# willi-menapace/PlayableVideoGeneration

Measured on AMD Instinct MI355X. Metric: training clips/sec (B x16x256x256), higher is better.
Workload: dtype f32; 1 GPU; bair256_t16_b8; variant=main, per_gpu_batch=8, global_batch=8, seq_len=16, gt_init=6, parallelism=dp1

## Files before the change

### include/caddy_hip.h

```cpp
#ifndef CADDY_HIP_H
#define CADDY_HIP_H
#include <stddef.h>
#ifdef __cplusplus
extern "C" {
#endif

typedef struct caddy_ctx caddy_ctx;

typedef struct caddy_config {
    int variant;
    int batch;
    int seq_len;
    int height, width;
    int stacking;
    int actions;
    int action_dim;
    int hidden;
    int use_gumbel, hard_gumbel, use_variations;
    float centroid_alpha;
    int perceptual;
    int ensemble;
} caddy_config;
#define CADDY_MAX_ENSEMBLE 8

// ... 123 lines not shown
int caddy_adam_step_ex(caddy_ctx* ctx, float* m, float* v, float lr, float beta1, float beta2, float eps, float weight_decay, int step, const int* member_step, int s2h_step,
                       float grad_scale);

int caddy_start_inference(caddy_ctx* ctx);
int caddy_f16_saturated(caddy_ctx* ctx);
int caddy_fallback_layers(caddy_ctx* ctx);
int caddy_generate_next(caddy_ctx* ctx, const float* observation, int action, const float* variation, float* frame_out, float* obs_out);

#define CADDY_PROFILE_FAMILIES 18
int caddy_debug_set_poison(caddy_ctx* ctx, int on);
int caddy_debug_set_seeds_only(caddy_ctx* ctx, int on);
int caddy_profile_begin(caddy_ctx* ctx);
int caddy_profile_end(caddy_ctx* ctx, double* out );
int caddy_profile_records(caddy_ctx* ctx, double* out, int max_records);
int caddy_profile_phases(caddy_ctx* ctx, char* names_out, float* ms_out, int max);

int caddy_debug_count(caddy_ctx* ctx);
int caddy_debug_fusion_counts(caddy_ctx* ctx, long* out3);
int caddy_debug_set_bn_paths(caddy_ctx* ctx, int small, int lazy, int epilogue_stats);
int caddy_debug_set_vgg_s16(caddy_ctx* ctx, int on);
int caddy_debug_set_s16_grads(caddy_ctx* ctx, int on);
int caddy_debug_set_perc_chunks(caddy_ctx* ctx, int n);
int caddy_debug_set_perc_fuse_l1(caddy_ctx* ctx, int on);
long caddy_debug_s16_grad_count(caddy_ctx* ctx);
int caddy_debug_set_pack_merged(caddy_ctx* ctx, int on);
int caddy_debug_dims(caddy_ctx* ctx, int i, int* nhwc4);
int caddy_debug_get(caddy_ctx* ctx, int i, int grad, float* dst_nchw);

int caddy_bn_layer_count(caddy_ctx* ctx);
long caddy_bn_calls(caddy_ctx* ctx, int i, char* name_out128);

struct ConvArgs; struct WgradArgs; struct PackDesc; struct TV;
int caddy_k_conv_fwd(const struct ConvArgs* a, void* stream);
int caddy_k_conv_wgrad(const struct WgradArgs* a, void* stream);
struct IgemmArgs;
size_t caddy_k_igemm_weight_bytes(int Cin, int Cout, int KH, int KW);
int caddy_k_igemm_pack(const float* w, const float* gamma, const float* beta, const float* mean, const float* var, float eps, const float* bias_in, int Cin, int Cout, int KH, int KW,
                       void* w32, void* w16, float* bias_out, void* stream);
int caddy_k_conv_igemm(const struct IgemmArgs* a, void* stream);
int caddy_k_fid_pool(const struct TV* in, const struct TV* out, int mode, void* stream);
int caddy_k_fid_global_avg(const struct TV* in, double* out, void* stream);
int caddy_k_fid_stage(const float* src, int n, int Hs, int Ws, float* out, int Ho, int Wo, void* stream);
struct Conv3dArgs; struct V5;
size_t caddy_k_conv3d_weight_bytes(int Cin, int Cout, int KT, int KH, int KW);
int caddy_k_conv3d_pack(const float* w_dhwio, const float* gamma, const float* beta, const float* mean, const float* var, float eps, const float* bias_in, int Cin, int Cout, int KT, int KH,
                        int KW, void* w32, void* w16, float* bias_out, void* stream);
// ... 25 lines not shown
```

### playablevideogeneration_amd/_lib.py

```python
import ctypes as C
import os

HERE = os.path.dirname(os.path.abspath(__file__))
LIB_PATH = os.path.join(HERE, "csrc", "libcaddy_hip.so")
CONV_MAX_SRC = 3
CONV_BK = 16


class TV(C.Structure):
    _fields_ = [("p", C.c_void_p), ("N", C.c_int), ("H", C.c_int), ("W", C.c_int), ("C", C.c_int), ("sn", C.c_long), ("ld", C.c_int), ("s16", C.c_int)]


class ConvSrc(C.Structure):
    _fields_ = [("p", C.c_void_p), ("sn", C.c_long), ("ld", C.c_int), ("C", C.c_int), ("Cpad", C.c_int), ("bcast", C.c_int),
                ("bn_scale", C.c_void_p), ("bn_shift", C.c_void_p), ("bn_act", C.c_int), ("bn_gn", C.c_int), ("bn_gs", C.c_long)]


class ConvArgs(C.Structure):
    _fields_ = [("src", ConvSrc * CONV_MAX_SRC), ("nsrc", C.c_int), ("N", C.c_int), ("H", C.c_int), ("W", C.c_int), ("KS", C.c_int),
                ("wp", C.c_void_p), ("Ktot", C.c_int), ("Cout", C.c_int), ("Cout_pad", C.c_int), ("bias", C.c_void_p), ("act", C.c_int),
                ("out", C.c_void_p), ("out_sn", C.c_long), ("out_ld", C.c_int), ("accumulate", C.c_int), ("precision", C.c_int), ("splitk", C.c_int), ("aux", C.c_void_p), ("split_scratch", C.c_void_p), ("split_cap", C.c_long), ("split_stride", C.c_long),
                ("mask", C.c_void_p), ("seed_ref", C.c_void_p), ("seed_w", C.c_float), ("wq", C.c_void_p), ("Kq", C.c_int), ("out_scale", C.c_float),
                ("res", C.c_void_p), ("res_sn", C.c_long), ("res_ld", C.c_int), ("xcd_map", C.c_int),
                ("pool_out", C.c_void_p), ("pool_sn", C.c_long), ("pool_ld", C.c_int), ("skip_out", C.c_int),
                ("stats", C.c_void_p), ("stats_ld", C.c_int), ("sat_flag", C.c_void_p), ("deterministic", C.c_int), ("direct_ok", C.c_int), ("lstm", C.c_void_p),
                ("in_s16", C.c_int), ("out_s16", C.c_int), ("pool_s16", C.c_int), ("mask_s16", C.c_int), ("seed_s16", C.c_int),
                ("avgpool", C.c_int), ("sat_out_next", C.c_int),
                ("l1_acc", C.c_void_p)]


class LstmFuse(C.Structure):
    _fields_ = [("cprev", C.c_void_p), ("cprev_sn", C.c_long), ("cprev_ld", C.c_int), ("h", C.c_void_p), ("h_sn", C.c_long), ("h_ld", C.c_int),
                ("c", C.c_void_p), ("c_sn", C.c_long), ("c_ld", C.c_int), ("hb", C.c_void_p), ("hb_sn", C.c_long), ("hb_ld", C.c_int),
                ("scale", C.c_void_p), ("shift", C.c_void_p), ("C", C.c_int)]


class WgradArgs(C.Structure):
    _fields_ = [("src", ConvSrc * CONV_MAX_SRC), ("nsrc", C.c_int), ("N", C.c_int), ("H", C.c_int), ("W", C.c_int), ("KS", C.c_int),
                ("dy", C.c_void_p), ("dy_sn", C.c_long), ("dy_ld", C.c_int), ("Cout", C.c_int), ("Cout_pad", C.c_int), ("Ktot", C.c_int),
                ("dwp", C.c_void_p), ("slabs", C.c_int), ("group_n", C.c_int), ("src_gs", C.c_long * CONV_MAX_SRC), ("dy_gs", C.c_long), ("precision", C.c_int),
                ("src_bn_gs", C.c_long * CONV_MAX_SRC), ("det_slab", C.c_void_p), ("det_cap", C.c_long), ("det_stride", C.c_long), ("dy_s16", C.c_int)]


class PackDesc(C.Structure):
    _fields_ = [("w", C.c_void_p * 4), ("gw", C.c_void_p * 4), ("nw", C.c_int), ("Co_each", C.c_int), ("Cin", C.c_int), ("KS", C.c_int),
                ("nseg", C.c_int), ("seg_off", C.c_int * CONV_MAX_SRC), ("seg_C", C.c_int * CONV_MAX_SRC), ("seg_Cpad", C.c_int * CONV_MAX_SRC),
                ("Cout", C.c_int), ("Cout_pad", C.c_int), ("Ktot", C.c_int), ("oscale", C.c_void_p)]


def round_up(a, b):
    return (a + b - 1) // b * b


_lib = None


def load(path=None):
    global _lib
    if path is None and _lib is not None:
        return _lib
    p = path or os.environ.get("CADDY_HIP_LIB") or LIB_PATH
    if not os.path.exists(p):
        raise RuntimeError(f"{p} not found: the HIP extension is not built (run __graft_entry__.build()); "
                           "playablevideogeneration_amd has no CPU fallback")
    lib = C.CDLL(p)
    if path is None:
        _lib = lib
    return lib
```

### playablevideogeneration_amd/csrc/common.h

```cpp
#pragma once
#include <hip/hip_runtime.h>
#include <cstdint>

typedef float f32x16 __attribute__((ext_vector_type(16)));
typedef float f32x4 __attribute__((ext_vector_type(4)));
typedef __bf16 bf16x8 __attribute__((ext_vector_type(8)));
typedef __bf16 bf16x4 __attribute__((ext_vector_type(4)));

struct TV {
    float* p;
    int N, H, W, C;
    long sn;
    int ld;
    int s16;
};

static inline int cdiv(long a, long b) { return (int)((a + b - 1) / b); }
static inline int round_up(int a, int b) { return (a + b - 1) / b * b; }

#define CONV_MAX_SRC 3
#define CONV_BK 16
struct ConvSrc {
    const float* p;
    long sn;
// ... 35 lines not shown
    int Kq;
    float out_scale;
    const float* res;
    long res_sn;
    int res_ld;
    int xcd_map;
    float* pool_out;
    long pool_sn;
    int pool_ld;
    int skip_out;
    float* stats;
    int stats_ld;
    unsigned* sat_flag;
    int deterministic;
    int direct_ok;
    const struct LstmFuse* lstm;
    int in_s16;
    int out_s16;
    int pool_s16;
    int mask_s16, seed_s16;
    int avgpool;
    int sat_out_next;
    double* l1_acc;
};
int conv_avgpool_ok(const ConvArgs& a);
struct LstmFuse { const float* cprev; long cprev_sn; int cprev_ld; float* h; long h_sn; int h_ld; float* c; long c_sn; int c_ld; float* hb; long hb_sn; int hb_ld; const float* scale; const float* shift; int C; };
extern thread_local int g_last_conv_lstm_fused;
#define HX_WSCALE 64.0f
enum { PREC_FP32 = 0, PREC_F16X3 = 16, PREC_BF16X3 = 17, PREC_F16X1 = 18, PREC_BF16X1 = 19 };
#define HX_KC 32
constexpr int CONV_AUX_BYTES = 128 * 1024;

struct WgradArgs {
    ConvSrc src[CONV_MAX_SRC];
    int nsrc;
    int N, H, W;
    int KS;
    const float* dy;
    long dy_sn;
    int dy_ld;
    int Cout, Cout_pad;
    int Ktot;
    float* dwp;
    int slabs;
    int group_n;
    long src_gs[CONV_MAX_SRC];
// ... 57 lines not shown
```

### playablevideogeneration_amd/csrc/conv_hx.hip

```cpp
#include "conv_hx_common.h"
#include "pack.h"
#include "pack_elems.h"
#include <cstdlib>

namespace {

template <typename T> __device__ __forceinline__ unsigned s16_bits(T h) { unsigned short s; __builtin_memcpy(&s, &h, 2); return s; }
template <typename T> __device__ __forceinline__ unsigned s16_pair(float v, int lane) {
    const T hi = (T)v;
    const T lo = (T)(v - (float)hi);
    const unsigned u = s16_bits(hi) | (s16_bits(lo) << 16);
    const unsigned w = (unsigned)__builtin_amdgcn_mov_dpp((int)u, 0xB1 , 0xF, 0xF, true);
    return (lane & 1) ? ((w >> 16) | (u & 0xffff0000u)) : ((u & 0xffffu) | (w << 16));
}
__device__ __forceinline__ int s16_slot(int col) { return (col & ~31) | ((col & 31) >> 1) | ((col & 1) << 4); }
__device__ __forceinline__ float s16_hi(const float* row, int col) { return (float)reinterpret_cast<const _Float16*>(row + (col & ~31))[col & 31]; }
__device__ __forceinline__ float s16_val(const float* row, int col) {
    const _Float16* h = reinterpret_cast<const _Float16*>(row + (col & ~31));
    return (float)h[col & 31] + (float)h[32 + (col & 31)];
}

template <typename T, int TH, int TW, int BN, int WM, int WN, int EP, bool SO, bool INTR, int MODE, int TMt, int TNt>
__device__ __forceinline__ void hx_epilogue(f32x16 (&acc)[TMt][TNt], float (&st1)[TNt], float (&st2)[TNt], unsigned& amax_o, double& l1s, const ConvArgs& a,
                                            int n, int n0, int y0, int x0, int lane, int wave) {
    constexpr bool E_POOL = EP == 1 || EP == 3, E_MASK = EP == 2 || EP == 3;
    constexpr int BM = TH * TW, RW = BM / WM / TW;
    const int wm_u = __builtin_amdgcn_readfirstlane(wave) / WN, wn = wave % WN;
    const int yw = y0 + wm_u * RW, xl = x0 + 4 * (lane >> 5);
    const int nx = a.W - xl;
    const bool masked = MODE == 1 || MODE == 3 || (MODE == 2 && E_MASK && a.mask != nullptr);
    const bool split = MODE == 2 && a.splitk > 1, slabs = split && a.split_stride != 0, atomics = split && !slabs;
    const bool with_res = MODE == 2 && !split && a.res != nullptr, accum = MODE == 2 && !split && a.accumulate != 0;
    char* const op = reinterpret_cast<char*>(a.out + (long)n * a.out_sn + (slabs ? (long)blockIdx.z * a.split_stride : 0L));
    const char* const mp = masked ? reinterpret_cast<const char*>(a.mask + (long)n * a.out_sn) : nullptr;
    const char* const sp = (masked && a.seed_ref) ? reinterpret_cast<const char*>(a.seed_ref + (long)n * a.out_sn) : nullptr;
    const char* const rp = with_res ? reinterpret_cast<const char*>(a.res + (long)n * a.res_sn) : nullptr;
    const unsigned ldb = (unsigned)a.out_ld * 4u, wldb = (unsigned)a.W * ldb;
// ... 62 lines not shown
                        if (EP == 0 && !split) { st1[j] += v; st2[j] = fmaf(v, v, st2[j]); }
                        const unsigned o_ = cb + HX_EOFF(i, r, wldb, ldb);
                        if (SO) {
                            if (!is_bf16<T>::value) { amax_o = max(amax_o, __float_as_uint(v) & 0x7fffffffu); v = __builtin_amdgcn_fmed3f(v, -HX_F16_MAX, HX_F16_MAX); if (E_POOL) acc[i][j][r] = v; }
                            const unsigned w_ = s16_pair<T>(v, lane);
                            if (store_full) *reinterpret_cast<unsigned*>(op + o_) = w_;
                        } else if (atomics) atomicAdd(reinterpret_cast<float*>(op + o_), v);
                        else if (store_full) *reinterpret_cast<float*>(op + o_) = v;
                    }
                }
                if (E_POOL && a.pool_out) {
                    char* const pp = reinterpret_cast<char*>(a.pool_out + (long)n * a.pool_sn);
                    const unsigned plb = (unsigned)a.pool_ld * 4u;
                    const int py = (yw + i * 2) >> 1;
                    const unsigned pb0 = (unsigned)(py * (a.W >> 1) + (xl >> 1)) * plb + ((SO && a.pool_s16) ? (unsigned)s16_slot(col) : (unsigned)col) * 4u;
#pragma unroll
                    for (int r = 0; r < 8; r += 2) {
                        const int pdx = ((r & 3) + 8 * ((r >> 2) & 1)) >> 1;
                        if (!INTR && (py >= (a.H >> 1) || (xl >> 1) + pdx >= (a.W >> 1))) continue;
                        const float mx = fmaxf(fmaxf(acc[i][j][r], acc[i][j][r + 1]), fmaxf(acc[i][j][r + 8], acc[i][j][r + 9]));
                        const unsigned po_ = pb0 + (unsigned)pdx * plb;
                        if (SO && a.pool_s16) *reinterpret_cast<unsigned*>(pp + po_) = s16_pair<T>(mx, lane);
                        else *reinterpret_cast<float*>(pp + po_) = mx;
                    }
                }
            }
        }
    }
#undef HX_EOFF
#undef HX_EOK
}

template <typename T, int NPL, int TH, int TW, int BN, int WM, int WN, int D, int EP = 0, int IO = 0, int BG = 0>
__global__ __launch_bounds__(64 * WM * WN) void k_conv_hx(ConvArgs a, int tiles_x, int tiles_y) {
    typedef typename Vec<T>::v8 v8;
    typedef typename Vec<T>::v4 v4;
    constexpr int NT = 64 * WM * WN;
    constexpr bool E_POOL = EP == 1 || EP == 3, E_MASK = EP == 2 || EP == 3;
    constexpr bool PS = (IO & 1) != 0, SO = (IO & 2) != 0;
    static_assert(!(PS || SO) || NPL == 2, "S16 tensors carry both halves");
    constexpr int BM = TH * TW;
    constexpr int HW_ = TW + 2, HH_ = TH + 2, HPX = HW_ * HH_;
    constexpr int PITCH = NPL * KC + 8;
    constexpr int AROW = (HW_ * PITCH + 127) / 128 * 128;
    constexpr int APP = NT / 8;
    constexpr int NA = (HPX + APP - 1) / APP;
// ... 484 lines not shown
    return true;
}
thread_local int g_last_conv_stats_tiles = 0;
thread_local int g_last_conv_direct = 0;

int conv_hx_avgpool_ok(const ConvArgs& a0) {
    ConvArgs a = a0;
    a.avgpool = 1;
    return conv_hx_try(a, nullptr, true) == 1 ? 1 : 0;
}

int conv_hx_try(const ConvArgs& a0, hipStream_t st, bool dry) {
    ConvArgs a = a0;
    if (a.KS != 3 || !a.wq || a.precision < PREC_F16X3 || a.precision > PREC_BF16X1 || a.act == 1) return 0;
    int kq = 0;
    for (int s = 0; s < a.nsrc; s++) { if ((a.src[s].ld & 3) || (a.src[s].sn & 3)) return -1; kq += round_up(a.src[s].C, HX_KC); }
    a.Kq = kq;
    a.out_scale = (a.precision == PREC_F16X3 || a.precision == PREC_F16X1) ? 1.0f / HX_WSCALE : 1.0f;
    int bn = hx_pick_bn(a.Cout);
    a.Cout_pad = round_up(a.Cout, bn);
    if (a.mask && a.accumulate) return -1;
    if (a.l1_acc && !conv_hx_l1_ok(a)) return -1;
    if (a.pool_out && (a.accumulate || a.mask)) return -1;
    if (a.avgpool) {
        if ((a.H | a.W) & 1 || a.accumulate || a.mask || a.pool_out || a.skip_out || a.stats || a.lstm || a.precision != PREC_F16X3 || a.in_s16 || a.out_s16) return dry ? 0 : -1;
        if (a.direct_ok && conv_direct_try(a, st, dry) == 1) {
            if (!dry) { g_last_conv_kernel = CK_HX_32; g_last_conv_stats_tiles = 0; g_last_conv_direct = 1; }
            return 1;
        }
    }
    if ((long)a.H * a.W * a.out_ld >= (1L << 30) || (a.res && (long)a.H * a.W * a.res_ld >= (1L << 30))) return 0;
    const int nchunks = kq / HX_KC;
    if (bn == 128 && g_hx_big_override < 0 && !a.pool_out && !a.skip_out && !a.mask &&
        (long)a.N * cdiv(a.W, 16) * cdiv(a.H, 8) * (a.Cout_pad / 128) <= 256) bn = 64;
    const int force_big = g_hx_big_override;
    bool big = bn == 128 && (long)a.N * cdiv(a.W, 16) * cdiv(a.H, 16) * (a.Cout_pad / bn) >= 384;
    if (force_big >= 0) big = bn == 128 && force_big == 1;
    const bool small_tiles = bn < 128 && force_big != 1 && (long)a.N * cdiv(a.W, 16) * cdiv(a.H, 16) * (a.Cout_pad / bn) < 384;
    const long blocks8 = (long)a.N * cdiv(a.W, 16) * cdiv(a.H, 8) * (a.Cout_pad / bn);
    const bool th4 = bn == 64 && small_tiles && !a.pool_out && !a.skip_out && !a.mask && !a.stats && blocks8 < 200 &&
                     ((a.direct_ok && a.precision == PREC_F16X3 && !a.accumulate) || a.precision == PREC_BF16X3);
    const int th = th4 ? 4 : ((bn == 128 && !big) || small_tiles) ? 8 : 16;
    const int tx = cdiv(a.W, 16), ty = cdiv(a.H, th);
    const long blocks = (long)a.N * tx * ty * (a.Cout_pad / bn);
    g_last_conv_direct = 0;
    if (!dry && !a.avgpool && a.direct_ok && blocks < 200 && conv_direct_try(a, st) == 1) { g_last_conv_kernel = CK_HX_32; g_last_conv_stats_tiles = 0; g_last_conv_direct = 1; return 1; }
// ... 107 lines not shown
```

### playablevideogeneration_amd/csrc/net.cpp

```cpp
#include "net.h"
#include "fid.h"
#include "fvd.h"
#include <cmath>
#include <cstdio>
#include <cstdlib>
#include <cstring>

static thread_local std::string g_err;
int finish(caddy_ctx* c, const char* sizer) {
    if (!c->dry && c->act.overflow() && !c->fail) { c->fail = true; g_err = std::string("activation arena overflow (workspace smaller than ") + sizer + ")"; }
    if (!c->dry) {
        hipError_t e = hipGetLastError();
        if (e != hipSuccess && !c->fail) { c->fail = true; g_err = std::string("HIP error: ") + hipGetErrorString(e); }
    }
    return c->fail ? -1 : 0;
}
void set_error(const std::string& s) { g_err = s; }
extern "C" const char* caddy_last_error(void) { return g_err.c_str(); }

#define RUN(expr) do { if (!dry) ck((expr), #expr); } while (0)

void caddy_ctx::ck(int rc, const char* what) {
    if (rc != 0 && !fail) { fail = true; set_error(std::string("kernel launch failed: ") + what); }
}
// ... 1451 lines not shown
    delete c;
}
size_t caddy_workspace_bytes(const caddy_config* cfg) {
    if (!check_cfg(cfg)) return 0;
    size_t p, a; dry_sizes(cfg, &p, &a);
    return p + 2 * a + 4096;
}
caddy_ctx* caddy_ctx_create(const caddy_config* cfg, float* params, float* grads, void* workspace, size_t workspace_bytes) {
    if (!check_cfg(cfg)) return nullptr;
    if (!params || !grads || !workspace) { set_error("null buffer"); return nullptr; }
    size_t p, a; dry_sizes(cfg, &p, &a);
    if (workspace_bytes < p + 2 * a) { set_error("workspace too small (see caddy_workspace_bytes)"); return nullptr; }
    if (((uintptr_t)workspace & 255) || ((uintptr_t)params & 15) || ((uintptr_t)grads & 15)) { set_error("buffers must be 256-byte (workspace) / 16-byte (params, grads) aligned"); return nullptr; }
    caddy_ctx* c = make_ctx(cfg, params, grads, workspace, a);
    if (c->fail) { delete c; return nullptr; }
    if (caddy_serial_streams()) c->use_dstream = false;
    hipMemset(c->sat_flag, 0, sizeof(unsigned) * 2 * CADDY_N_FLAGS);
    if (const char* e = getenv("CADDY_DETERMINISTIC")) c->deterministic = atoi(e) != 0;
    if (const char* e = getenv("CADDY_PERC_CHUNKS")) { const int n = atoi(e); if (n < 0) c->perc_chunks_force = -n; else c->perc_chunks_cfg = n; }
    if (const char* e = getenv("CADDY_MASK_FROM_X")) c->mask_from_x = atoi(e) != 0;
    if (const char* e = getenv("CADDY_S16_GRADS")) c->s16_grads = atoi(e) != 0;
    if (const char* e = getenv("CADDY_VGG_S16")) c->vgg_s16 = atoi(e) != 0;
    if (const char* e = getenv("CADDY_PERC_FUSE_L1")) c->perc_fuse_l1 = atoi(e) != 0;
    if (const char* e = getenv("CADDY_PRECISION")) {
        if (!strcmp(e, "exact") || !strcmp(e, "0")) { c->prec_fwd = c->prec_bwd = PREC_FP32; c->vgg_precision = c->vgg_precision_bwd = PREC_FP32; }
        else if (!strcmp(e, "fwd")) { c->prec_bwd = PREC_FP32; c->vgg_precision_bwd = PREC_FP32; }
    }
    return c;
}
extern "C" int caddy_dp_shutdown(caddy_ctx* c);
void caddy_ctx_destroy(caddy_ctx* c) {
    if (c && (c->comm || c->comm2)) caddy_dp_shutdown(c);
    if (c && c->side) { hipStreamSynchronize(c->side); hipStreamDestroy(c->side); }
    if (c) for (int k = 0; k < caddy_ctx::PERC_MAX_CHUNKS; k++) if (c->perc_ev[k]) hipEventDestroy(c->perc_ev[k]);
    if (c && c->gstream) { if (c->graph_exec) hipStreamSynchronize(c->stream); hipStreamSynchronize(c->gstream); c->drop_graph(); hipStreamDestroy(c->gstream); }
    if (c) for (ConvL* L : c->convs) if (L->off_ev) hipEventDestroy(L->off_ev);
    if (c && c->dstream) { hipStreamSynchronize(c->dstream); hipStreamDestroy(c->dstream); if (c->d_done) hipEventDestroy(c->d_done); }
    fid_free(c);
    fvd_free(c);
    delete c;
}
int caddy_set_stream(caddy_ctx* c, void* s) { c->stream = (hipStream_t)s; return 0; }
int caddy_debug_set_poison(caddy_ctx* c, int on) { c->poison_nz = on != 0; return 0; }
int caddy_debug_set_bn_paths(caddy_ctx* c, int small, int lazy, int epilogue_stats) { c->bn_small = small != 0; c->lazy_bn = lazy != 0; c->epi_stats = epilogue_stats != 0; return 0; }
int caddy_debug_set_vgg_s16(caddy_ctx* c, int on) { c->vgg_s16 = on != 0; return 0; }
int caddy_debug_set_s16_grads(caddy_ctx* c, int on) { c->s16_grads = on != 0; return 0; }
int caddy_debug_set_perc_chunks(caddy_ctx* c, int n) { c->perc_chunks_force = n; return 0; }
int caddy_debug_set_perc_fuse_l1(caddy_ctx* c, int on) { c->perc_fuse_l1 = on != 0; return 0; }
long caddy_debug_s16_grad_count(caddy_ctx* c) { long n = 0; for (const GradFmt& g : c->gfmts) n += g.fmt ? 1 : 0; return n; }
int caddy_debug_set_pack_merged(caddy_ctx* c, int on) { c->merged_pack = on != 0; c->pack_jobs.key = -1; for (auto& j : c->unpack_jobs) j.key = -1; return 0; }
int caddy_debug_set_seeds_only(caddy_ctx* c, int on) { c->seeds_only = on != 0; return 0; }
int caddy_set_grads_ready_hook(caddy_ctx* c, caddy_grads_ready_hook hook, void* user) { c->grads_hook = hook; c->grads_user = user; return 0; }
int caddy_set_sampler_hook(caddy_ctx* c, caddy_sampler_hook hook, void* user, int provides_samples, int provides_variations) {
    c->samplers = SamplerHooks{};
    if (hook && (provides_samples || provides_variations)) { c->samplers.fn = hook; c->samplers.user = user; c->samplers.action = provides_samples; c->samplers.variation = provides_variations; }
    return 0;
}
int caddy_set_allreduce_hook(caddy_ctx* c, void (*hook)(float*, int, void*), void* user, int world_size) {
    c->hook = hook; c->hook_user = user; c->world = world_size > 1 ? world_size : 1;
    return 0;
}
int caddy_forward_full(caddy_ctx* c, const float* obs, int gt_init, float tau, const caddy_noise* noise, int training, const float* samples_in, const float* variations_in) {
    if (!ctx_needs(c, CTX_MODEL, "caddy_forward_full")) return -2;
    c->fail = false;
    if (!obs || !noise) { set_error("null input"); return -2; }
    return forward_full(c, obs, gt_init, tau, noise, training, samples_in, variations_in);
}
int caddy_forward_pretraining(caddy_ctx* c, const float* obs, float tau, const caddy_noise* noise, int training, const float* samples_in, const float* variations_in) {
    if (!ctx_needs(c, CTX_MODEL, "caddy_forward_pretraining")) return -2;
    c->fail = false;
    if (!obs || !noise) { set_error("null input"); return -2; }
// ... 166 lines not shown
```

### playablevideogeneration_amd/csrc/net.h

```cpp
#pragma once
#include <algorithm>
#include <array>
#include <deque>
#include <functional>
#include <string>
#include <vector>
#include "caddy_hip.h"
#include "common.h"
#include "head.h"
#include "pack.h"
#include "pointwise.h"
#include "perceptual.h"

struct GradFmt { bool elig; int fmt; };
struct T4 {
    float* d; float* g;
    int N, H, W, C; long sn; int ld;
    bool nz = false;
    bool nz2 = false;
    const float* bn_scale = nullptr; const float* bn_shift = nullptr; int bn_act = 0;
    int fmt = 0;
    GradFmt* gs = nullptr;
};
static inline TV dv(const T4& t) { return TV{t.d, t.N, t.H, t.W, t.C, t.sn, t.ld, 0}; }
// ... 111 lines not shown
    void (*grads_hook)(float* grads, long offset, long count, void* stream, void* user) = nullptr; void* grads_user = nullptr;
    long bucket_lo[2] = {0, 0}, bucket_hi[2] = {0, 0}; bool lstm_early_done = false;
    long s2h_lo = 0, s2h_hi = 0;
    void early_gradient_buckets();
    void* comm = nullptr; void* comm2 = nullptr;
    int comm_world = 1; std::vector<std::pair<long, long>> comm_buckets; hipStream_t comm_bucket_stream = nullptr;
    SamplerHooks samplers{};
    bool deterministic = true;
    float* wgrad_det = nullptr; long wgrad_det_cap = 0;
    hipStream_t wgrad_det_owner = nullptr; bool wgrad_det_owner_set = false;
    long n_pool_fallback = 0;
    long n_wgrad_det_handover = 0;
    unsigned* sat_flag = nullptr;
    bool layer_fallback[CADDY_N_FLAGS] = {false};
    int n_fallback = 0;
    float* conv_split = nullptr; long conv_split_cap = 0;
    float* conv_aux = nullptr;
    float* conv_aux2 = nullptr;
    double* red_scratch = nullptr;
    VggState vgg;
    int vgg_precision = PREC_F16X3, vgg_precision_bwd = PREC_BF16X3;
    bool vgg_s16 = true;
    bool perc_fuse_l1 = true;
    int prec_fwd = PREC_F16X3, prec_bwd = PREC_BF16X3;
    T4 gt_img[3]{}; size_t gt_scratch_off = 0, gt_scratch_end = 0; bool gt_prefetched = false, perc_prefetch = true; hipEvent_t gt_done = nullptr;
    static constexpr int PERC_MAX_CHUNKS = 8;
    int perc_chunks_cfg = 3;
    int perc_chunks_force = 0;
    int perc_nch = 1, perc_trec = 0;
    int perc_t0[PERC_MAX_CHUNKS + 1] = {};
    hipEvent_t perc_ev[PERC_MAX_CHUNKS] = {};
    bool perc_waited[PERC_MAX_CHUNKS] = {};
    bool perc_pipelined = false;
    T4 gt_taps_c[PERC_MAX_CHUNKS][3][5]{};
    bool perc_range(int r, int k, int* t0, int* len) const {
        if (r == 0 || perc_nch == 1) { if (r != 0 && k != 0) return false; *t0 = r == 0 ? perc_t0[k + 1] : 0; *len = r == 0 ? perc_t0[k] - perc_t0[k + 1] : perc_trec; return true; }
        const int kb = perc_nch / 2;
        if (k == 0) { *t0 = perc_t0[kb]; *len = perc_trec - perc_t0[kb]; return true; }
        if (k == kb) { *t0 = 0; *len = perc_t0[kb]; return true; }
        return false;
    }
    void perc_plan(int Trec, bool chunked);
    void perc_wait(int t);
    size_t gt_lo = 0, gt_hi = 0;
    size_t fwd_off = 0;
    int prof_kind_override = -1;
// ... 93 lines not shown
```

### playablevideogeneration_amd/csrc/perceptual.hip

```cpp
#include "net.h"
#include "perceptual.h"
#include "lpips.h"
#include <cstdio>
#include <cstring>

#define RUN_CK(c, expr) do { if (!(c)->dry) (c)->ck((expr), #expr); } while (0)

namespace {

const VggSpec VGG19_SPEC[VGG_NCONV] = {
    {0, 3, 64, 0, 0}, {2, 64, 64, 0, -1}, {5, 64, 128, 1, 1}, {7, 128, 128, 0, -1}, {10, 128, 256, 1, 2}, {12, 256, 256, 0, -1}, {14, 256, 256, 0, -1},
    {16, 256, 256, 0, -1}, {19, 256, 512, 1, 3}, {21, 512, 512, 0, -1}, {23, 512, 512, 0, -1}, {25, 512, 512, 0, -1}, {28, 512, 512, 1, 4}};
const VggSpec LPIPS_SPEC[VGG_NCONV] = {
    {0, 3, 64, 0, -1}, {2, 64, 64, 0, 0}, {5, 64, 128, 1, -1}, {7, 128, 128, 0, 1}, {10, 128, 256, 1, -1}, {12, 256, 256, 0, -1}, {14, 256, 256, 0, 2},
    {17, 256, 512, 1, -1}, {19, 512, 512, 0, -1}, {21, 512, 512, 0, 3}, {24, 512, 512, 1, -1}, {26, 512, 512, 0, -1}, {28, 512, 512, 0, 4}};
const int LPIPS_C[5] = {64, 128, 256, 512, 512};

__global__ __launch_bounds__(256) void k_maxpool2(const float* in, float* out, long n_out4, int Hi, int Wi, int C4) {
    const int Ho = Hi >> 1, Wo = Wi >> 1;
    for (long i = blockIdx.x * 256L + threadIdx.x; i < n_out4; i += (long)gridDim.x * 256) {
        int c = (int)(i % C4); long q = i / C4; int x = (int)(q % Wo); q /= Wo; int y = (int)(q % Ho); long n = q / Ho;
        const float4* p = reinterpret_cast<const float4*>(in) + ((n * Hi + 2 * y) * (long)Wi + 2 * x) * C4 + c;
        float4 a = p[0], b = p[C4], d = p[(long)Wi * C4], e = p[(long)Wi * C4 + C4];
        float4 m;
// ... 30 lines not shown
}
template <bool AS, bool ZS>
__global__ __launch_bounds__(256) void k_maxpool2_bwd_relu(const float* a, const float* gp, float* gz, long n_win4, int Hi, int Wi, int C4) {
    const int Ho = Hi >> 1, Wo = Wi >> 1, Hc = (Hi + 1) >> 1, Wc = (Wi + 1) >> 1;
    for (long i = blockIdx.x * 256L + threadIdx.x; i < n_win4; i += (long)gridDim.x * 256) {
        int c = (int)(i % C4); long q = i / C4; int x = (int)(q % Wc); q /= Wc; int y = (int)(q % Hc); long n = q / Hc;
        const long base = ((n * Hi + 2 * y) * (long)Wi + 2 * x) * C4 + c;
        const long o1 = C4, o2 = (long)Wi * C4, o3 = o2 + C4;
        if (y >= Ho || x >= Wo) {
            const float4 zero = make_float4(0.f, 0.f, 0.f, 0.f);
            st4_grad<ZS>(gz, base, zero);
            if (2 * x + 1 < Wi) st4_grad<ZS>(gz, base + o1, zero);
            if (2 * y + 1 < Hi) { st4_grad<ZS>(gz, base + o2, zero); if (2 * x + 1 < Wi) st4_grad<ZS>(gz, base + o3, zero); }
            continue;
        }
        const float4 A = ld4<AS>(a, base), B = ld4<AS>(a, base + o1), D = ld4<AS>(a, base + o2), E = ld4<AS>(a, base + o3);
        const float4 G = reinterpret_cast<const float4*>(gp)[((n * Ho + y) * (long)Wo + x) * C4 + c];
        float4 zA, zB, zD, zE;
        route4(A.x, B.x, D.x, E.x, G.x, zA.x, zB.x, zD.x, zE.x);
        route4(A.y, B.y, D.y, E.y, G.y, zA.y, zB.y, zD.y, zE.y);
        route4(A.z, B.z, D.z, E.z, G.z, zA.z, zB.z, zD.z, zE.z);
        route4(A.w, B.w, D.w, E.w, G.w, zA.w, zB.w, zD.w, zE.w);
        st4_grad<ZS>(gz, base, zA); st4_grad<ZS>(gz, base + o1, zB); st4_grad<ZS>(gz, base + o2, zD); st4_grad<ZS>(gz, base + o3, zE);
    }
}
template <bool RS, bool GS, bool ZS>
__global__ __launch_bounds__(256) void k_feat_l1(const float* rec, const float* gt, long n4, float seed_w, float* gz, double* acc) {
    __shared__ double sh[4];
    double s = 0.0;
    for (long i = blockIdx.x * 256L + threadIdx.x; i < n4; i += (long)gridDim.x * 256) {
        const float4 r = ld4<RS>(rec, i), g = ld4<GS>(gt, i);
        const float d[4] = {r.x - g.x, r.y - g.y, r.z - g.z, r.w - g.w};
        const float rv[4] = {r.x, r.y, r.z, r.w};
        float z[4];
#pragma unroll
        for (int e = 0; e < 4; e++) {
            s += (double)fabsf(d[e]);
            z[e] = rv[e] > 0.f ? (d[e] > 0.f ? seed_w : (d[e] < 0.f ? -seed_w : 0.f)) : 0.f;
        }
        if (gz) st4_grad<ZS>(gz, i, make_float4(z[0], z[1], z[2], z[3]));
    }
    for (int o = 32; o > 0; o >>= 1) s += __shfl_xor(s, o);
    if ((threadIdx.x & 63) == 0) sh[threadIdx.x >> 6] = s;
    __syncthreads();
    if (threadIdx.x == 0) atomicAdd(acc, sh[0] + sh[1] + sh[2] + sh[3]);
}
// ... 110 lines not shown
    const float* r = rec.d; const float* t = gt.d;
    if (rec.fmt && gt.fmt) hipLaunchKernelGGL((k_feat_l1_img<true, true>), g, b, 0, st, r, t, n4, acc);
    else if (rec.fmt) hipLaunchKernelGGL((k_feat_l1_img<true, false>), g, b, 0, st, r, t, n4, acc);
    else if (gt.fmt) hipLaunchKernelGGL((k_feat_l1_img<false, true>), g, b, 0, st, r, t, n4, acc);
    else hipLaunchKernelGGL((k_feat_l1_img<false, false>), g, b, 0, st, r, t, n4, acc);
}
int cos_blocks(const T4& f) { const long n4 = (long)f.H * f.W * (f.C / 4); return (int)(n4 / 1024 < 1 ? 1 : (n4 / 1024 > 64 ? 64 : n4 / 1024)); }
void launch_feat_cos_img(hipStream_t st, const T4& x, const T4& y, double* part) {
    const long n4 = (long)x.H * x.W * (x.C / 4);
    const dim3 g(cos_blocks(x), x.N), b(256);
    if (x.fmt && y.fmt) hipLaunchKernelGGL((k_feat_cos_img<true, true>), g, b, 0, st, x.d, y.d, n4, part);
    else if (x.fmt) hipLaunchKernelGGL((k_feat_cos_img<true, false>), g, b, 0, st, x.d, y.d, n4, part);
    else if (y.fmt) hipLaunchKernelGGL((k_feat_cos_img<false, true>), g, b, 0, st, x.d, y.d, n4, part);
    else hipLaunchKernelGGL((k_feat_cos_img<false, false>), g, b, 0, st, x.d, y.d, n4, part);
}
void launch_maxpool_bwd(hipStream_t st, const T4& pre, const float* gp, bool gz_s16) {
    const long n4 = (long)pre.N * ((pre.H + 1) / 2) * ((pre.W + 1) / 2) * (pre.C / 4);
    const dim3 g(grid_for(n4)), b(256);
    const float* a = pre.d;
    if (pre.fmt && gz_s16) hipLaunchKernelGGL((k_maxpool2_bwd_relu<true, true>), g, b, 0, st, a, gp, pre.g, n4, pre.H, pre.W, pre.C / 4);
    else if (pre.fmt) hipLaunchKernelGGL((k_maxpool2_bwd_relu<true, false>), g, b, 0, st, a, gp, pre.g, n4, pre.H, pre.W, pre.C / 4);
    else if (gz_s16) hipLaunchKernelGGL((k_maxpool2_bwd_relu<false, true>), g, b, 0, st, a, gp, pre.g, n4, pre.H, pre.W, pre.C / 4);
    else hipLaunchKernelGGL((k_maxpool2_bwd_relu<false, false>), g, b, 0, st, a, gp, pre.g, n4, pre.H, pre.W, pre.C / 4);
}
}

const VggSpec* vgg_spec_table(int kind) { return kind == VGG_KIND_LPIPS ? LPIPS_SPEC : VGG19_SPEC; }
static long spec_param_floats(const VggSpec* VS) {
    long n = 0;
    for (int i = 0; i < VGG_NCONV; i++) n += (long)VS[i].cout * VS[i].cin * 9 + round_up(VS[i].cout, 4);
    return n;
}
static int spec_param_info(const VggSpec* VS, int index, caddy_param_info* out) {
    if (index < 0 || index >= 2 * VGG_NCONV) return -1;
    long off = 0;
    for (int i = 0; i < VGG_NCONV; i++) {
        const long nw = (long)VS[i].cout * VS[i].cin * 9;
        if (index == 2 * i || index == 2 * i + 1) {
            memset(out, 0, sizeof(*out));
            const bool w = index == 2 * i;
            snprintf(out->name, sizeof(out->name), "features.%d.%s", VS[i].idx, w ? "weight" : "bias");
            out->offset = w ? off : off + nw; out->kind = 3;
            if (w) { out->ndim = 4; out->shape[0] = VS[i].cout; out->shape[1] = VS[i].cin; out->shape[2] = 3; out->shape[3] = 3; }
            else { out->ndim = 1; out->shape[0] = VS[i].cout; out->shape[1] = out->shape[2] = out->shape[3] = 1; }
            return 0;
        }
// ... 54 lines not shown
        VggLayer& L = V.conv[i];
        const long nw = (long)VS[i].cout * VS[i].cin * 9;
        L.pd.w[0] = flat + off;
        RUN_CK(c, pack_fwd(L.pd, L.wp, c->stream));
        RUN_CK(c, pack_dgrad(L.pd, 0, L.wpd, L.cd_pad, L.kd, c->stream));
        for (int pl = 0; pl < 2; pl++) {
            RUN_CK(c, pack_hx(L.pd, L.wq[pl], round_up(L.pd.Cout, hx_pick_bn(L.pd.Cout)), -1, pl == 0 ? PREC_F16X3 : PREC_F16X1, c->stream));
            if (L.wqd[pl]) RUN_CK(c, pack_hx(L.pd, L.wqd[pl], round_up(VS[i].cin, hx_pick_bn(VS[i].cin)), 0, pl == 0 ? PREC_BF16X3 : PREC_BF16X1, c->stream));
        }
        RUN_CK(c, pack_hx(L.pd, L.wq[2], round_up(L.pd.Cout, hx_pick_bn(L.pd.Cout)), -1, PREC_BF16X3, c->stream));
        if (!dry) hipLaunchKernelGGL(k_copy_f, dim3(1), dim3(256), 0, c->stream, flat + off + nw, L.bias, (long)VS[i].cout);
        L.pd.w[0] = nullptr;
        off += nw + round_up(VS[i].cout, 4);
    }
    if (V.kind == VGG_KIND_LPIPS) for (int l = 0; l < 5; l++) {
        if (!dry) hipLaunchKernelGGL(k_copy_f, dim3(1), dim3(256), 0, c->stream, flat + off, V.lin[l], (long)LPIPS_C[l]);
        off += LPIPS_C[l];
    }
    V.loaded = true;
    return c->fail ? -1 : 0;
}

namespace {
struct Branch { T4 a[VGG_NCONV]; T4 p[VGG_NCONV]; };

int conv_call(caddy_ctx* c, const ConvArgs& a, double flops, int kind) {
    int save = c->prof_kind_override;
    c->prof_kind_override = kind;
    int rc = c->timed_conv_fwd(a, flops);
    c->prof_kind_override = save;
    return rc;
}
bool vgg_use_s16(const caddy_ctx* c) { return c->vgg_s16 && c->vgg_precision == PREC_F16X3 && c->vgg_precision_bwd == PREC_BF16X3; }
bool vgg_io_ok(const caddy_ctx* c, int i, int N, int H, int W) {
    const VggSpec* VS = c->vgg.spec;
    return vgg_use_s16(c) && VS[i].cin >= 32 && !c->layer_fallback[CADDY_VGG_FLAG0 + i] && conv_hx_s16_ok(N, H, W, VS[i].cout);
}

void vgg_forward(caddy_ctx* c, const T4& img, Branch& B, const T4* taps, bool keep_all) {
    bool dry = c->dry;
    VggState& V = c->vgg;
    const VggSpec* VS = V.spec;
    T4 x = img;
    T4 pooled{};
    bool have_pooled = false;
    for (int i = 0; i < VGG_NCONV; i++) {
        VggLayer& L = V.conv[i];
// ... 5 lines not shown
                if (x.fmt) { c->fail = true; set_error("internal: S16 feature map handed to the stand-alone max-pool"); }
                if (!dry) hipLaunchKernelGGL(k_maxpool2, dim3(grid_for(n4)), dim3(256), 0, c->stream, (const float*)x.d, p.d, n4, x.H, x.W, p.C / 4);
                B.p[i] = p; x = p;
            }
        }
        T4 out = (taps && VS[i].tap >= 0) ? taps[VS[i].tap] : valloc(c, x.N, x.H, x.W, VS[i].cout);
        out.fmt = 0;
        ConvArgs a{};
        a.src[0] = ConvSrc{x.d, x.sn, x.ld, x.C, round_up(x.C, CONV_BK), 0};
        a.nsrc = 1; a.N = x.N; a.H = x.H; a.W = x.W; a.KS = 3; a.wp = L.wp; a.Ktot = L.pd.Ktot; a.Cout = L.pd.Cout; a.Cout_pad = L.pd.Cout_pad;
        a.bias = L.bias; a.act = 2; a.out = out.d; a.out_sn = out.sn; a.out_ld = out.ld;
        a.precision = c->vgg_precision == PREC_F16X1 ? PREC_F16X1 : (c->vgg_precision == PREC_FP32 ? PREC_FP32 : (c->vgg_precision == PREC_BF16X3 ? PREC_BF16X3 : PREC_F16X3));
        if (a.precision == PREC_F16X3 && c->layer_fallback[CADDY_VGG_FLAG0 + i]) a.precision = PREC_BF16X3;
        if (a.precision != PREC_FP32) a.wq = L.wq[a.precision == PREC_F16X1 ? 1 : (a.precision == PREC_BF16X3 ? 2 : 0)];
        a.sat_flag = c->sat_flag + CADDY_VGG_FLAG0 + i;
        const bool io_here = vgg_io_ok(c, i, x.N, x.H, x.W);
        const bool pool_next = i + 1 < VGG_NCONV && VS[i + 1].pool_before;
        a.in_s16 = x.fmt;
        if (x.fmt && !io_here) { c->fail = true; set_error("internal: S16 input for a VGG19 launch that cannot read it"); }
        if (pool_next && a.wq && a.precision == PREC_F16X3 && VS[i].cin >= 32 && conv_hx_pool_ok(x.N, x.H, x.W, VS[i].cout)) {
            pooled = valloc(c, x.N, x.H / 2, x.W / 2, VS[i].cout);
            a.pool_out = pooled.d; a.pool_sn = pooled.sn; a.pool_ld = pooled.ld;
            a.skip_out = (!keep_all && VS[i].tap < 0) ? 1 : 0;
            have_pooled = true;
            if (io_here && vgg_io_ok(c, i + 1, x.N, x.H / 2, x.W / 2)) { a.pool_s16 = 1; pooled.fmt = 1; if (!a.skip_out) { a.out_s16 = 1; out.fmt = 1; } }
        } else if (io_here && !pool_next) {
            if (i + 1 == VGG_NCONV || vgg_io_ok(c, i + 1, x.N, x.H, x.W)) { a.out_s16 = 1; out.fmt = 1; }
        }
        a.sat_out_next = ((a.out_s16 || a.pool_s16) && i + 1 < VGG_NCONV) ? 1 : 0;
        if (!dry) c->ck(conv_call(c, a, 2.0 * x.N * x.H * x.W * 9.0 * VS[i].cin * VS[i].cout, 3), "vgg conv");
        B.a[i] = out; x = out;
    }
}
}

void vgg_gt_prefetch(caddy_ctx* c, int Trec, int t_off) {
    bool dry = c->dry;
    const caddy_config& g = c->cfg;
    const VggSpec* VS = c->vgg.spec;
    const int tc[5] = {64, 128, 256, 512, 512};
    c->perc_plan(Trec, c->training && !c->pretraining);
    c->gt_lo = (c->act.off + 255) & ~(size_t)255;
    T4 gimg[caddy_ctx::PERC_MAX_CHUNKS][3];
    int kmax = 0;
    for (int k = 0; k < c->perc_nch; k++) {
        if (c->perc_t0[k] - c->perc_t0[k + 1] > c->perc_t0[kmax] - c->perc_t0[kmax + 1]) kmax = k;
// ... 36 lines not shown
            const long npix = (long)gi.N * gi.H * gi.W;
            hipLaunchKernelGGL(k_gt_resize, dim3(grid_for(npix)), dim3(256), 0, side, dv(c->obs), gi.d, gi.H, gi.W, npix, 1 << r, t_off + t0, g.seq_len, len);
            const size_t keep = c->act.off;
            c->act.off = c->gt_scratch_off;
            Branch G{};
            vgg_forward(c, gi, G, c->gt_taps_c[k][r], false);
            for (int i = 0; i < VGG_NCONV; i++) if (VS[i].tap >= 0) c->gt_taps_c[k][r][VS[i].tap].fmt = G.a[i].fmt;
            c->act.off = keep;
        }
    }
    c->stream = main_st;
    hipEventRecord(c->gt_done, side);
    c->gt_prefetched = true;
}

void vgg_perceptual(caddy_ctx* c, double lambda, const T4* gt_img, VggLevels* lv) {
    bool dry = c->dry;
    VggState& V = c->vgg;
    const VggSpec* VS = V.spec;
    hipStream_t st = c->stream;
    const caddy_config& g = c->cfg;
    const bool pre = c->gt_prefetched && !dry;
    const int nch = c->perc_nch, Trec = c->perc_trec, B = g.batch;
    const bool pipe = c->perc_pipelined && nch > 1 && !dry;
    const bool no_par = caddy_serial_streams();
    const bool par = nch == 1 && !no_par && !dry && c->use_side && c->side != nullptr && !c->prof;
    hipStream_t side = (par || pipe) ? c->wgrad_stream() : st;
    if (pre) { hipStreamWaitEvent(st, c->gt_done, 0); if (pipe) hipStreamWaitEvent(side, c->gt_done, 0); }
    const size_t mark_all = c->act.off;
    size_t side_end = mark_all;
    size_t side_base = mark_all;
    for (int k = 0; k < nch; k++) {
    const bool first_par = nch > 1 && k == 0 && (pipe || dry);
    for (int oi = 0; oi < 3; oi++) {
        const int r = first_par ? oi : (oi == 2 ? 0 : oi + 1);
        int t0, len;
        if (!c->perc_range(r, k, &t0, &len)) continue;
        const bool whole = len == Trec;
        const bool on_side = (pipe && !(first_par && r == 0)) || (par && r != 0);
        c->stream = on_side ? side : st;
        hipStream_t st = c->stream;
        float* const aux = on_side ? c->conv_aux2 : c->conv_aux;
        if (nch > 1) c->act.off = (first_par && r == 0) ? mark_all : side_base;
        else if (r == 0 && !no_par) c->act.off = side_end;
        const T4& full = c->frames[r];
        const size_t mark = c->act.off;
// ... 53 lines not shown
                    d.mask = in.d; d.mask_s16 = in.fmt;
                    if (VS[i - 1].tap >= 0) { const T4& tp = taps[VS[i - 1].tap]; d.seed_ref = tp.d; d.seed_w = wl[VS[i - 1].tap]; d.seed_s16 = tp.fmt; }
                    d.out_s16 = gzs[i - 1] ? 1 : 0;
                }
                return d;
        };
        bool l1_fused[5] = {false, false, false, false, false};
        for (int l = 0; l < 5; l++) {
            const T4& f = R.a[li[l]];
            double* const lacc = c->loss_acc + LOSS_PERC_R0 + 6 * r + 1 + l;
            if (l < 4 && lambda != 0.0 && c->perc_fuse_l1 && li[l] + 1 < VGG_NCONV && !VS[li[l] + 1].pool_before) {
                const ConvArgs d = dgrad_args(li[l] + 1);
                l1_fused[l] = d.seed_ref != nullptr && conv_hx_l1_ok(d);
            }
            if (!dry && !l1_fused[l]) launch_feat_l1(st, f, taps[l], wl[l], l == 4 ? f.g : (float*)nullptr, gzs[li[4]], lacc);
        }
        if (lambda != 0.0) {
            for (int i = VGG_NCONV - 1; i >= 0; i--) {
                const T4& in = VS[i].pool_before ? R.p[i] : (i > 0 ? R.a[i - 1] : rec);
                ConvArgs d = dgrad_args(i);
                if (i > 0 && VS[i - 1].tap >= 0 && l1_fused[VS[i - 1].tap]) d.l1_acc = c->loss_acc + LOSS_PERC_R0 + 6 * r + 1 + VS[i - 1].tap;
                if (!dry) c->ck(conv_call(c, d, 2.0 * in.N * in.H * in.W * 9.0 * VS[i].cin * VS[i].cout, 4), "vgg dgrad");
                if (VS[i].pool_before) {
                    if (!dry) launch_maxpool_bwd(st, R.a[i - 1], (const float*)in.g, gzs[i - 1]);
                }
            }
            if (!whole && !dry)
                hipLaunchKernelGGL(k_time_chunk, dim3(grid_for((long)rec.N * F4)), dim3(256), 0, st, (float4*)full.g, (float4*)rec.g, F4, Trec, t0, len, (long)rec.N * F4, 1);
        }
        if (r != 0 && c->act.off > side_end) side_end = c->act.off;
        if (nch == 1) c->act.off = mark;
        if (first_par && r == 0) side_base = c->act.off;
    }
    if (pipe) hipEventRecord(c->perc_ev[k], side);
    }
    c->stream = st;
    if (par) {
        hipEvent_t e = c->sev();
        hipEventRecord(e, side);
        hipStreamWaitEvent(st, e, 0);
    }
    c->act.off = mark_all;
}

int vgg_eval_per_frame(caddy_ctx* c, double* out_host) {
    const caddy_config& g = c->cfg;
    if (!g.perceptual || !c->vgg.loaded) { set_error("caddy_perceptual_per_frame needs a context created with caddy_config.perceptual = 1 and loaded VGG19 weights"); return -2; }
// ... 96 lines not shown
```

Measured before the change: 67.76 clips/s.

## Store maxpool argmax indices in VGG forward and route pool backward through them

For untapped pooled VGG layers kept for backward, the fused conv+pool epilogue now writes a one-byte argmax/positive-sign index per pooled element into the (otherwise skipped) full-resolution output buffer, instead of writing the full pre-pool activation. The backward maxpool then uses a new kernel that scatters the pooled gradient via these indices rather than rereading the full-resolution activations to recompute the argmax. This is meant to cut forward store traffic and backward read bandwidth for those layers. It adds per-element compare logic in the epilogue and s16 round-trip emulation to keep tie behaviour consistent with the stored format.

```diff
diff --git a/include/caddy_hip.h b/include/caddy_hip.h
--- a/include/caddy_hip.h
+++ b/include/caddy_hip.h
@@ -169,6 +169,9 @@
 int caddy_debug_set_s16_grads(caddy_ctx* ctx, int on);
 int caddy_debug_set_perc_chunks(caddy_ctx* ctx, int n);
 int caddy_debug_set_perc_fuse_l1(caddy_ctx* ctx, int on);
+int caddy_debug_set_perc_pool_idx(caddy_ctx* ctx, int on);
+int caddy_debug_set_frames(caddy_ctx* ctx, int r, const float* src_nchw);
+int caddy_debug_pool_route_counts(caddy_ctx* ctx, long* out2);
 long caddy_debug_s16_grad_count(caddy_ctx* ctx);
 int caddy_debug_set_pack_merged(caddy_ctx* ctx, int on);
 int caddy_debug_dims(caddy_ctx* ctx, int i, int* nhwc4);
diff --git a/playablevideogeneration_amd/_lib.py b/playablevideogeneration_amd/_lib.py
--- a/playablevideogeneration_amd/_lib.py
+++ b/playablevideogeneration_amd/_lib.py
@@ -26,7 +26,8 @@
                 ("stats", C.c_void_p), ("stats_ld", C.c_int), ("sat_flag", C.c_void_p), ("deterministic", C.c_int), ("direct_ok", C.c_int), ("lstm", C.c_void_p),
                 ("in_s16", C.c_int), ("out_s16", C.c_int), ("pool_s16", C.c_int), ("mask_s16", C.c_int), ("seed_s16", C.c_int),
                 ("avgpool", C.c_int), ("sat_out_next", C.c_int),
-                ("l1_acc", C.c_void_p)]
+                ("l1_acc", C.c_void_p),
+                ("pool_idx", C.c_void_p)]
 
 
 class LstmFuse(C.Structure):
@@ -64,6 +65,10 @@
         raise RuntimeError(f"{p} not found: the HIP extension is not built (run __graft_entry__.build()); "
                            "playablevideogeneration_amd has no CPU fallback")
     lib = C.CDLL(p)
+    if hasattr(lib, "caddy_debug_set_perc_pool_idx"):
+        lib.caddy_debug_set_perc_pool_idx.argtypes = [C.c_void_p, C.c_int]
+        lib.caddy_debug_pool_route_counts.argtypes = [C.c_void_p, C.POINTER(C.c_long)]
+        lib.caddy_debug_set_frames.argtypes = [C.c_void_p, C.c_int, C.c_void_p]
     if path is None:
         _lib = lib
     return lib
diff --git a/playablevideogeneration_amd/csrc/common.h b/playablevideogeneration_amd/csrc/common.h
--- a/playablevideogeneration_amd/csrc/common.h
+++ b/playablevideogeneration_amd/csrc/common.h
@@ -81,6 +81,7 @@
     int avgpool;
     int sat_out_next;
     double* l1_acc;
+    unsigned char* pool_idx;
 };
 int conv_avgpool_ok(const ConvArgs& a);
 struct LstmFuse { const float* cprev; long cprev_sn; int cprev_ld; float* h; long h_sn; int h_ld; float* c; long c_sn; int c_ld; float* hb; long hb_sn; int hb_ld; const float* scale; const float* shift; int C; };
diff --git a/playablevideogeneration_amd/csrc/conv_hx.hip b/playablevideogeneration_amd/csrc/conv_hx.hip
--- a/playablevideogeneration_amd/csrc/conv_hx.hip
+++ b/playablevideogeneration_amd/csrc/conv_hx.hip
@@ -13,6 +13,7 @@
     const unsigned w = (unsigned)__builtin_amdgcn_mov_dpp((int)u, 0xB1 , 0xF, 0xF, true);
     return (lane & 1) ? ((w >> 16) | (u & 0xffff0000u)) : ((u & 0xffffu) | (w << 16));
 }
+template <typename T> __device__ __forceinline__ float s16_round_trip(float v) { const T hi = (T)v; const T lo = (T)(v - (float)hi); return (float)hi + (float)lo; }
 __device__ __forceinline__ int s16_slot(int col) { return (col & ~31) | ((col & 31) >> 1) | ((col & 1) << 4); }
 __device__ __forceinline__ float s16_hi(const float* row, int col) { return (float)reinterpret_cast<const _Float16*>(row + (col & ~31))[col & 31]; }
 __device__ __forceinline__ float s16_val(const float* row, int col) {
@@ -121,6 +122,15 @@
                         const unsigned po_ = pb0 + (unsigned)pdx * plb;
                         if (SO && a.pool_s16) *reinterpret_cast<unsigned*>(pp + po_) = s16_pair<T>(mx, lane);
                         else *reinterpret_cast<float*>(pp + po_) = mx;
+                        if (a.pool_idx) {
+                            float c0 = acc[i][j][r], c1 = acc[i][j][r + 1], c2 = acc[i][j][r + 8], c3 = acc[i][j][r + 9];
+                            if (SO && a.pool_s16) { c0 = s16_round_trip<T>(c0); c1 = s16_round_trip<T>(c1); c2 = s16_round_trip<T>(c2); c3 = s16_round_trip<T>(c3); }
+                            unsigned k_ = 0u; float m_ = c0;
+                            if (c1 > m_) { m_ = c1; k_ = 1u; }
+                            if (c2 > m_) { m_ = c2; k_ = 2u; }
+                            if (c3 > m_) { m_ = c3; k_ = 3u; }
+                            a.pool_idx[(long)n * a.pool_sn + (unsigned)(py * (a.W >> 1) + (xl >> 1) + pdx) * (unsigned)a.pool_ld + (unsigned)col] = (unsigned char)(k_ | (m_ > 0.f ? 4u : 0u));
+                        }
                     }
                 }
             }
@@ -651,6 +661,7 @@
     if (a.mask && a.accumulate) return -1;
     if (a.l1_acc && !conv_hx_l1_ok(a)) return -1;
     if (a.pool_out && (a.accumulate || a.mask)) return -1;
+    if (a.pool_idx && !a.pool_out) return -1;
     if (a.avgpool) {
         if ((a.H | a.W) & 1 || a.accumulate || a.mask || a.pool_out || a.skip_out || a.stats || a.lstm || a.precision != PREC_F16X3 || a.in_s16 || a.out_s16) return dry ? 0 : -1;
         if (a.direct_ok && conv_direct_try(a, st, dry) == 1) {
diff --git a/playablevideogeneration_amd/csrc/net.cpp b/playablevideogeneration_amd/csrc/net.cpp
--- a/playablevideogeneration_amd/csrc/net.cpp
+++ b/playablevideogeneration_amd/csrc/net.cpp
@@ -1497,6 +1497,7 @@
     if (const char* e = getenv("CADDY_S16_GRADS")) c->s16_grads = atoi(e) != 0;
     if (const char* e = getenv("CADDY_VGG_S16")) c->vgg_s16 = atoi(e) != 0;
     if (const char* e = getenv("CADDY_PERC_FUSE_L1")) c->perc_fuse_l1 = atoi(e) != 0;
+    if (const char* e = getenv("CADDY_PERC_POOL_IDX")) c->perc_pool_idx = atoi(e) != 0;
     if (const char* e = getenv("CADDY_PRECISION")) {
         if (!strcmp(e, "exact") || !strcmp(e, "0")) { c->prec_fwd = c->prec_bwd = PREC_FP32; c->vgg_precision = c->vgg_precision_bwd = PREC_FP32; }
         else if (!strcmp(e, "fwd")) { c->prec_bwd = PREC_FP32; c->vgg_precision_bwd = PREC_FP32; }
@@ -1522,6 +1523,13 @@
 int caddy_debug_set_s16_grads(caddy_ctx* c, int on) { c->s16_grads = on != 0; return 0; }
 int caddy_debug_set_perc_chunks(caddy_ctx* c, int n) { c->perc_chunks_force = n; return 0; }
 int caddy_debug_set_perc_fuse_l1(caddy_ctx* c, int on) { c->perc_fuse_l1 = on != 0; return 0; }
+int caddy_debug_set_perc_pool_idx(caddy_ctx* c, int on) { c->perc_pool_idx = on != 0; return 0; }
+int caddy_debug_set_frames(caddy_ctx* c, int r, const float* src_nchw) {
+    if (!c->have_forward || r < 0 || r > 2 || !c->frames[r].d) { set_error("caddy_debug_set_frames: no forward results / unknown resolution"); return -2; }
+    const T4& t = c->frames[r];
+    return pw_nchw_to_nhwc(src_nchw, (long)t.C * t.H * t.W, dv(t), c->stream);
+}
+int caddy_debug_pool_route_counts(caddy_ctx* c, long* out2) { out2[0] = c->pool_route_n[0]; out2[1] = c->pool_route_n[1]; return 0; }
 long caddy_debug_s16_grad_count(caddy_ctx* c) { long n = 0; for (const GradFmt& g : c->gfmts) n += g.fmt ? 1 : 0; return n; }
 int caddy_debug_set_pack_merged(caddy_ctx* c, int on) { c->merged_pack = on != 0; c->pack_jobs.key = -1; for (auto& j : c->unpack_jobs) j.key = -1; return 0; }
 int caddy_debug_set_seeds_only(caddy_ctx* c, int on) { c->seeds_only = on != 0; return 0; }
diff --git a/playablevideogeneration_amd/csrc/net.h b/playablevideogeneration_amd/csrc/net.h
--- a/playablevideogeneration_amd/csrc/net.h
+++ b/playablevideogeneration_amd/csrc/net.h
@@ -157,6 +157,8 @@
     int vgg_precision = PREC_F16X3, vgg_precision_bwd = PREC_BF16X3;
     bool vgg_s16 = true;
     bool perc_fuse_l1 = true;
+    bool perc_pool_idx = true;
+    long pool_route_n[2] = {0, 0};
     int prec_fwd = PREC_F16X3, prec_bwd = PREC_BF16X3;
     T4 gt_img[3]{}; size_t gt_scratch_off = 0, gt_scratch_end = 0; bool gt_prefetched = false, perc_prefetch = true; hipEvent_t gt_done = nullptr;
     static constexpr int PERC_MAX_CHUNKS = 8;
diff --git a/playablevideogeneration_amd/csrc/perceptual.hip b/playablevideogeneration_amd/csrc/perceptual.hip
--- a/playablevideogeneration_amd/csrc/perceptual.hip
+++ b/playablevideogeneration_amd/csrc/perceptual.hip
@@ -76,6 +76,50 @@
         route4(A.z, B.z, D.z, E.z, G.z, zA.z, zB.z, zD.z, zE.z);
         route4(A.w, B.w, D.w, E.w, G.w, zA.w, zB.w, zD.w, zE.w);
         st4_grad<ZS>(gz, base, zA); st4_grad<ZS>(gz, base + o1, zB); st4_grad<ZS>(gz, base + o2, zD); st4_grad<ZS>(gz, base + o3, zE);
+    }
+}
+typedef __bf16 bf16x8_t __attribute__((ext_vector_type(8)));
+template <bool S> __device__ __forceinline__ void st8_grad(float* p, long i, const float (&v)[8]) {
+    if (S) {
+        __bf16* h = reinterpret_cast<__bf16*>(p + ((8 * i) & ~31L)) + ((8 * i) & 31);
+        bf16x8_t hi, lo;
+#pragma unroll
+        for (int e = 0; e < 8; e++) { hi[e] = (__bf16)v[e]; lo[e] = (__bf16)(v[e] - (float)hi[e]); }
+        *reinterpret_cast<bf16x8_t*>(h) = hi;
+        *reinterpret_cast<bf16x8_t*>(h + 32) = lo;
+    } else {
+        reinterpret_cast<float4*>(p)[2 * i] = make_float4(v[0], v[1], v[2], v[3]);
+        reinterpret_cast<float4*>(p)[2 * i + 1] = make_float4(v[4], v[5], v[6], v[7]);
+    }
+}
+template <bool ZS>
+__global__ __launch_bounds__(256) void k_maxpool2_bwd_idx(const unsigned char* idx, const float* gp, float* gz, long n_win8, int Hi, int Wi, int C8) {
+    const int Ho = Hi >> 1, Wo = Wi >> 1, Hc = (Hi + 1) >> 1, Wc = (Wi + 1) >> 1;
+    for (long i = blockIdx.x * 256L + threadIdx.x; i < n_win8; i += (long)gridDim.x * 256) {
+        int c = (int)(i % C8); long q = i / C8; int x = (int)(q % Wc); q /= Wc; int y = (int)(q % Hc); long n = q / Hc;
+        const long base = ((n * Hi + 2 * y) * (long)Wi + 2 * x) * C8 + c;
+        const long o1 = C8, o2 = (long)Wi * C8, o3 = o2 + C8;
+        float z[4][8];
+        if (y >= Ho || x >= Wo) {
+#pragma unroll
+            for (int e = 0; e < 8; e++) z[0][e] = 0.f;
+            st8_grad<ZS>(gz, base, z[0]);
+            if (2 * x + 1 < Wi) st8_grad<ZS>(gz, base + o1, z[0]);
+            if (2 * y + 1 < Hi) { st8_grad<ZS>(gz, base + o2, z[0]); if (2 * x + 1 < Wi) st8_grad<ZS>(gz, base + o3, z[0]); }
+            continue;
+        }
+        const long pw = ((n * Ho + y) * (long)Wo + x) * C8 + c;
+        const float4 G0 = reinterpret_cast<const float4*>(gp)[2 * pw], G1 = reinterpret_cast<const float4*>(gp)[2 * pw + 1];
+        const unsigned long long K = reinterpret_cast<const unsigned long long*>(idx)[pw];
+        const float g[8] = {G0.x, G0.y, G0.z, G0.w, G1.x, G1.y, G1.z, G1.w};
+#pragma unroll
+        for (int e = 0; e < 8; e++) {
+            const unsigned b = (unsigned)(K >> (8 * e)) & 0xffu;
+            const int k = (int)(b & 3u);
+            const float v = (b & 4u) ? g[e] : 0.f;
+            z[0][e] = k == 0 ? v : 0.f; z[1][e] = k == 1 ? v : 0.f; z[2][e] = k == 2 ? v : 0.f; z[3][e] = k == 3 ? v : 0.f;
+        }
+        st8_grad<ZS>(gz, base, z[0]); st8_grad<ZS>(gz, base + o1, z[1]); st8_grad<ZS>(gz, base + o2, z[2]); st8_grad<ZS>(gz, base + o3, z[3]);
     }
 }
 template <bool RS, bool GS, bool ZS>
@@ -232,6 +276,12 @@
     else if (pre.fmt) hipLaunchKernelGGL((k_maxpool2_bwd_relu<true, false>), g, b, 0, st, a, gp, pre.g, n4, pre.H, pre.W, pre.C / 4);
     else if (gz_s16) hipLaunchKernelGGL((k_maxpool2_bwd_relu<false, true>), g, b, 0, st, a, gp, pre.g, n4, pre.H, pre.W, pre.C / 4);
     else hipLaunchKernelGGL((k_maxpool2_bwd_relu<false, false>), g, b, 0, st, a, gp, pre.g, n4, pre.H, pre.W, pre.C / 4);
+}
+void launch_maxpool_bwd_idx(hipStream_t st, const T4& pre, const unsigned char* idx, const float* gp, bool gz_s16) {
+    const long n8 = (long)pre.N * ((pre.H + 1) / 2) * ((pre.W + 1) / 2) * (pre.C / 8);
+    const dim3 g(grid_for(n8)), b(256);
+    if (gz_s16) hipLaunchKernelGGL((k_maxpool2_bwd_idx<true>), g, b, 0, st, idx, gp, pre.g, n8, pre.H, pre.W, pre.C / 8);
+    else hipLaunchKernelGGL((k_maxpool2_bwd_idx<false>), g, b, 0, st, idx, gp, pre.g, n8, pre.H, pre.W, pre.C / 8);
 }
 }
 
@@ -332,7 +382,7 @@
 }
 
 namespace {
-struct Branch { T4 a[VGG_NCONV]; T4 p[VGG_NCONV]; };
+struct Branch { T4 a[VGG_NCONV]; T4 p[VGG_NCONV]; const unsigned char* pidx[VGG_NCONV]; };
 
 int conv_call(caddy_ctx* c, const ConvArgs& a, double flops, int kind) {
     int save = c->prof_kind_override;
@@ -384,6 +434,10 @@
             pooled = valloc(c, x.N, x.H / 2, x.W / 2, VS[i].cout);
             a.pool_out = pooled.d; a.pool_sn = pooled.sn; a.pool_ld = pooled.ld;
             a.skip_out = (!keep_all && VS[i].tap < 0) ? 1 : 0;
+            if (keep_all && c->perc_pool_idx && VS[i].tap < 0 && (VS[i].cout & 7) == 0) {
+                a.pool_idx = reinterpret_cast<unsigned char*>(out.d); a.skip_out = 1;
+                B.pidx[i] = a.pool_idx;
+            }
             have_pooled = true;
             if (io_here && vgg_io_ok(c, i + 1, x.N, x.H / 2, x.W / 2)) { a.pool_s16 = 1; pooled.fmt = 1; if (!a.skip_out) { a.out_s16 = 1; out.fmt = 1; } }
         } else if (io_here && !pool_next) {
@@ -466,6 +520,7 @@
     const caddy_config& g = c->cfg;
     const bool pre = c->gt_prefetched && !dry;
     const int nch = c->perc_nch, Trec = c->perc_trec, B = g.batch;
+    if (!dry) c->pool_route_n[0] = c->pool_route_n[1] = 0;
     const bool pipe = c->perc_pipelined && nch > 1 && !dry;
     const bool no_par = caddy_serial_streams();
     const bool par = nch == 1 && !no_par && !dry && c->use_side && c->side != nullptr && !c->prof;
@@ -565,7 +620,10 @@
                 if (i > 0 && VS[i - 1].tap >= 0 && l1_fused[VS[i - 1].tap]) d.l1_acc = c->loss_acc + LOSS_PERC_R0 + 6 * r + 1 + VS[i - 1].tap;
                 if (!dry) c->ck(conv_call(c, d, 2.0 * in.N * in.H * in.W * 9.0 * VS[i].cin * VS[i].cout, 4), "vgg dgrad");
                 if (VS[i].pool_before) {
-                    if (!dry) launch_maxpool_bwd(st, R.a[i - 1], (const float*)in.g, gzs[i - 1]);
+                    if (!dry) {
+                        if (R.pidx[i - 1]) { launch_maxpool_bwd_idx(st, R.a[i - 1], R.pidx[i - 1], (const float*)in.g, gzs[i - 1]); c->pool_route_n[0]++; }
+                        else { launch_maxpool_bwd(st, R.a[i - 1], (const float*)in.g, gzs[i - 1]); c->pool_route_n[1]++; }
+                    }
                 }
             }
             if (!whole && !dry)
```

Result: no change. 67.96 clips/s (median of 6 runs) (+0.3%).
